# yc015/fully-automated-multi-heartbeat-echocardiography-video-segmentation-and-motion-tracking

Measured on AMD Instinct MI355X. Metric: 32f×112×112 clips/sec at 1/2/4/8 MI355X; Dice Δ vs CPU ref, higher is better.
Workload: dtype fp32

## Files before the change

### fully-automated-multi-heartbeat-echocardiography-video-segmentation-and-motion-tracking_amd/_lib.py

```python
import ctypes
import os

from .build import LIB_PATH

c_int, c_int64, c_void_p, c_char_p = ctypes.c_int, ctypes.c_int64, ctypes.c_void_p, ctypes.c_char_p
_P = c_void_p

SIGNATURES = {
    "clasfv_last_error": (c_char_p, []),
    "clasfv_version": (c_int, []),
    "clasfv_source_hash": (c_char_p, []),
    "clasfv_create": (c_int, [c_int, ctypes.POINTER(c_void_p)]),
    "clasfv_destroy": (c_int, [_P]),
    "clasfv_param_count": (c_int, [_P]),
    "clasfv_param_info": (c_int, [_P, c_int, ctypes.POINTER(c_char_p), ctypes.POINTER(c_int), ctypes.POINTER(c_int64)]),
    "clasfv_load_param": (c_int, [_P, c_char_p, _P, c_int64]),
    "clasfv_finalize": (c_int, [_P]),
    "clasfv_forward": (c_int, [_P, _P, c_int, c_int, c_int, c_int, _P, _P, _P]),
    "clasfv_workspace_bytes": (c_int64, [_P]),
    "clasfv_set_compute_dtype": (c_int, [_P, c_int]),
    "clasfv_get_compute_dtype": (c_int, [_P]),
    "clasfv_set_kernel_variants": (c_int, [_P, c_int]),
    "clasfv_get_kernel_variants": (c_int, [_P]),
    "clasfv_set_kernel_timing": (c_int, [_P, c_int]),
    "clasfv_kernel_timing": (c_int, [_P, c_int, ctypes.POINTER(c_char_p), ctypes.POINTER(c_int),
                                     ctypes.POINTER(ctypes.c_double), ctypes.POINTER(ctypes.c_double),
                                     ctypes.POINTER(ctypes.c_double)]),
    "clasfv_set_launch_log": (c_int, [_P, c_int]),
    "clasfv_launch_log": (c_int, [_P, c_int, ctypes.POINTER(c_char_p), ctypes.POINTER(c_int64), ctypes.POINTER(c_int),
                                  ctypes.POINTER(c_int)]),
    "clasfv_fill_workspace": (c_int, [_P, c_int, _P]),
    "clasfv_conv_count": (c_int, [_P]),
    "clasfv_conv_info": (c_int, [_P, c_int, ctypes.POINTER(c_char_p), ctypes.POINTER(c_char_p), ctypes.POINTER(c_int),
                                 ctypes.POINTER(c_int), ctypes.POINTER(c_int), ctypes.POINTER(c_int),
                                 ctypes.POINTER(c_int), ctypes.POINTER(c_int), ctypes.POINTER(c_int)]),
    "clasfv_run_conv": (c_int, [_P, c_int, _P, c_int, c_int, c_int, c_int, _P, _P, c_int, c_int, c_int, _P, _P, c_int64,
                                ctypes.POINTER(c_char_p), _P]),
    "clasfv_run_decoder": (c_int, [_P, _P, _P, _P, _P, c_int, c_int, c_int, c_int, _P, _P, _P]),
    "clasfv_build_clips": (c_int, [_P, c_int, c_int, c_int, _P, c_int, c_int, _P, _P]),
    "clasfv_pass_labels": (c_int, [_P, c_int, _P, c_int, c_int, c_int, c_int, c_int, _P, _P]),
    "clasfv_pass_labels_margin": (c_int, [_P, c_int, _P, c_int, c_int, c_int, c_int, c_int, _P, _P]),
    "clasfv_logit_margin": (c_int, [_P, c_int, c_int, c_int, _P, _P]),
    "clasfv_fuse_votes": (c_int, [_P, c_int, c_int, c_int, c_int, c_int, c_int, _P, _P]),
    "clasfv_warp": (c_int, [_P, c_int, c_int, c_int, c_int, _P, c_int64, c_int64, _P, _P]),
    "clasfv_zeroone_workspace_bytes": (c_int64, []),
    "clasfv_zeroone_normalize": (c_int, [_P, c_int64, _P, _P]),
# ... 71 lines not shown
```

### fully-automated-multi-heartbeat-echocardiography-video-segmentation-and-motion-tracking_amd/csrc/common.h

```cpp
#pragma once
#include <hip/hip_runtime.h>
#include <stdint.h>

#include "clasfv.h"

typedef float f32x4 __attribute__((ext_vector_type(4)));
typedef float f32x2 __attribute__((ext_vector_type(2)));

__device__ inline float relu1(float x) { return __int_as_float(max(__float_as_int(x), 0)); }

__device__ inline f32x4 psub4(f32x4 a, f32x4 b) {
  const f32x2 alo = {a[0], a[1]}, ahi = {a[2], a[3]}, blo = {b[0], b[1]}, bhi = {b[2], b[3]};
  f32x2 lo, hi;
  asm("v_pk_add_f32 %0, %1, %2 neg_lo:[0,1] neg_hi:[0,1]" : "=v"(lo) : "v"(alo), "v"(blo));
  asm("v_pk_add_f32 %0, %1, %2 neg_lo:[0,1] neg_hi:[0,1]" : "=v"(hi) : "v"(ahi), "v"(bhi));
  return f32x4{lo[0], lo[1], hi[0], hi[1]};
}


struct FastDiv {
  unsigned m;
  int l;
};
inline FastDiv fast_div(unsigned d) {
// ... 25 lines not shown
  } while (0)
#define CLASFV_LAUNCH(kernel, grid, ...) CLASFV_LAUNCH_P(1, kernel, grid, __VA_ARGS__)

struct ConvParams {
  const void* x;
  const void* w;
  const float* bias;
  const void* res;
  void* y;
  int N, Ti, Hi, Wi, Cin;
  int To, Ho, Wo, Cout;
  int KT, KH, KW, st, sh, sw, pt, ph, pw;
  int K, Kp, M, relu;
  const void* zero;
  const void* x2;
  int Cin2;
  int stem;
  int in_bf16, out_bf16;
  int x_c8, y_c8;
  int vflags, patch_nt;
  float* part;
  int n_split;
};

struct DecTap {
  const float* p;
  int T, H, W;
  float st, sh, sw;
};

struct DecParams {
  DecTap tap[4];
  const float* b1;
  const float* w2;
  const void* w2x3;
  const float* b2;
  const float* wh;
  const float* bh;
  float* seg;
  float* mot;
  int N, T, H, W;
  int bf16;
  int x3;
  void* idx;
};
inline size_t decoder_index_bytes(int T, int H, int W) { return (size_t)4 * (T + H + W) * 16; }
// ... 53 lines not shown
```

### fully-automated-multi-heartbeat-echocardiography-video-segmentation-and-motion-tracking_amd/csrc/engine.hip

```cpp
#include <cxxabi.h>
#include <math.h>
#include <stdio.h>
#include <stdlib.h>
#include <string.h>

#include <string>
#include <unordered_map>
#include <vector>

#include "clasfv.h"
#include "common.h"
#include "plumbing.h"
#include "track.h"

namespace {

thread_local std::string g_err;

int fail(int code, const std::string& msg) {
  g_err = msg;
  return code;
}

#define HIP_TRY(expr)                                                                        \
// ... 136 lines not shown
  c.cout_p = c.role == PROJ ? c.cout : pad_channels(c.cout, bf16);
  c.K = c.kt * c.kh * c.kw * c.cin_p + c.cin2;
  c.Kp = round_up(c.K, c.in_bf16 ? 32 : 16);
  c.cout_alloc = c.cout_p;
}

Conv make_conv(Role role, const std::string& w, const std::string& bn, int cin, int cout, int kt, int kh, int kw,
               int st, int sh, int sw, int pt, int ph, int pw) {
  Conv c;
  c.role = role;
  c.w = w;
  c.bn = bn;
  c.cin = cin;
  c.cout = cout;
  c.kt = kt, c.kh = kh, c.kw = kw, c.st = st, c.sh = sh, c.sw = sw, c.pt = pt, c.ph = ph, c.pw = pw;
  layout_conv(c, false);
  return c;
}

int midplanes(int i, int o) { return (i * o * 27) / (i * 9 + 3 * o); }

struct Tuning {
  int vflags = 0, conv_nt = 0, patch_nt = 0;
};

}

struct clasfv_engine {
  int device = 0;
  std::vector<Param> params;
  std::unordered_map<std::string, int> index;
  std::vector<Conv> convs;
  Conv proj[5];
  float *b1 = nullptr, *w2 = nullptr, *b2 = nullptr, *wh = nullptr, *bh = nullptr;
  void* w2x3 = nullptr;
  bool ready = false;
  int dtype = CLASFV_DTYPE_FP32;
  Tuning tune;
  float* zero = nullptr;
  struct Ctx {
    hipStream_t stream = nullptr;
    char* arena = nullptr;
    size_t arena_bytes = 0;
    hipStream_t side = nullptr;
    hipEvent_t ev_fork = nullptr, ev_join = nullptr;
    uint64_t last_use = 0;
// ... 456 lines not shown

bool c8_pair(const Conv& a, const Conv& b, const Shape5& in, const Tuning& tu) {
  if (tu.vflags & CLASFV_VARIANT_NO_C8) return false;
  Shape5 mid, out;
  ConvParams pa = conv_params(a, in, mid);
  ConvParams pb = conv_params(b, mid, out);
  pa.vflags = pb.vflags = tu.vflags;
  return kKernels[pick_kernel(a, pa)].writes_c8 && !a.out_bf16 && kKernels[pick_kernel(b, pb)].reads_c8 &&
         winot_c8_ok(pb);
}

void split_k(ConvParams& p, int S, void* scratch, size_t scratch_bytes) {
  if (S > 1 && scratch && (size_t)S * p.M * p.Cout * sizeof(float) <= scratch_bytes) {
    p.part = reinterpret_cast<float*>(scratch);
    p.n_split = S;
  }
}

int run_conv(const Conv& c, const void* x, const Shape5& in, void* y, Shape5& out, const void* res, bool relu,
             hipStream_t s, const void* zero_block, const void* x2, const KernelInfo** kernel, const Tuning& tu,
             int x_c8 = 0, int y_c8 = 0, void* scratch = nullptr, size_t scratch_bytes = 0) {
  if (in.c != c.cin_p) return fail(CLASFV_EINVAL, "internal: channel mismatch");
  ConvParams p = conv_params(c, in, out);
  p.vflags = tu.vflags;
  p.patch_nt = tu.patch_nt;
  p.x = x;
  p.res = res;
  p.y = y;
  p.relu = relu ? 1 : 0;
  p.zero = zero_block;
  p.x2 = x2;
  p.x_c8 = x_c8;
  p.y_c8 = y_c8;
  const KernelInfo& k = kKernels[pick_kernel(c, p)];
  *kernel = &k;
  if ((y_c8 && !k.writes_c8) || (x_c8 && !k.reads_c8))
    return fail(CLASFV_EINVAL, "internal: 8-channel-blocked layout on an unsupported kernel");
  p.w = c.*k.image;
  switch (k.id) {
    case K_WINO4R: HIP_TRY(launch_wino4r(p, s)); break;
    case K_WINO4W: HIP_TRY(launch_wino4w(p, s)); break;
    case K_WINO4: HIP_TRY(launch_wino4(p, s)); break;
    case K_WINO_Q: HIP_TRY(launch_winoq(p, s)); break;
    case K_WINO: HIP_TRY(launch_wino(p, s)); break;
    case K_STEM_BF16: HIP_TRY(launch_stem_bf16(p, s)); break;
    case K_STEM_X3: HIP_TRY(launch_stem_x3(p, s)); break;
    case K_WINOT:
// ... 202 lines not shown
    h->log.push_back({it->second.c_str(), r.e[i].grid, r.e[i].passes, conv});
  }
}

}

extern "C" {

const char* clasfv_last_error(void) { return g_err.c_str(); }
int clasfv_version(void) { return CLASFV_ABI_VERSION; }
#ifndef CLASFV_SOURCE_HASH
#define CLASFV_SOURCE_HASH "unhashed"
#endif
const char* clasfv_source_hash(void) { return "clasfv-source-hash:" CLASFV_SOURCE_HASH; }

int clasfv_create(int device, clasfv_t* out) {
  if (!out) return fail(CLASFV_EINVAL, "null out");
  int n = 0;
  HIP_TRY(hipGetDeviceCount(&n));
  if (device < 0 || device >= n) return fail(CLASFV_EINVAL, "bad device index");
  auto* e = new clasfv_engine();
  e->device = device;
  e->tune.vflags = env_variants();
  e->tune.conv_nt = env_int("CLASFV_CONV_NT");
  e->tune.patch_nt = env_int("CLASFV_PATCH_NT");
  build_plan(e);
  *out = e;
  return CLASFV_OK;
}

int clasfv_destroy(clasfv_t h) {
  if (!h) return CLASFV_OK;
  DeviceGuard guard(h->device);
  for (auto& c : h->convs) free_conv_images(c);
  for (auto& c : h->proj) free_conv_images(c);
  for (auto* c : h->ctxs) {
    if (c->side) (void)hipStreamDestroy(c->side);
    if (c->ev_fork) (void)hipEventDestroy(c->ev_fork);
    if (c->ev_join) (void)hipEventDestroy(c->ev_join);
    (void)hipFree(c->arena);
    delete c;
  }
  (void)hipFree(h->b1);
  (void)hipFree(h->w2);
  (void)hipFree(h->w2x3);
  (void)hipFree(h->b2);
// ... 67 lines not shown
}

int clasfv_set_compute_dtype(clasfv_t h, int dtype) {
  if (!h) return fail(CLASFV_EINVAL, "null handle");
  if (dtype != CLASFV_DTYPE_FP32 && dtype != CLASFV_DTYPE_BF16) return fail(CLASFV_EINVAL, "unknown dtype");
  if (dtype != h->dtype) {
    h->dtype = dtype;
    h->ready = false;
  }
  return CLASFV_OK;
}

int clasfv_get_compute_dtype(clasfv_t h) { return h ? h->dtype : CLASFV_EINVAL; }

int clasfv_set_kernel_variants(clasfv_t h, int flags) {
  if (!h) return fail(CLASFV_EINVAL, "null handle");
  if (flags & ~kVariantMask) return fail(CLASFV_EINVAL, "unknown kernel-variant bit");
  if ((flags ^ h->tune.vflags) & CLASFV_VARIANT_NO_WINOGRAD) h->ready = false;
  h->tune.vflags = flags;
  return CLASFV_OK;
}

int clasfv_get_kernel_variants(clasfv_t h) { return h ? h->tune.vflags : CLASFV_EINVAL; }

int clasfv_forward(clasfv_t h, const float* x, int N, int T, int H, int W, float* seg, float* mot, void* stream) {
  if (!h) return fail(CLASFV_EINVAL, "null handle");
  if (!h->ready) return fail(CLASFV_ENOTREADY, "clasfv_finalize has not been called");
  if (!x || !seg || !mot) return fail(CLASFV_EINVAL, "null tensor");
  if (N < 1) return fail(CLASFV_EINVAL, "N must be >= 1");
  if (T < 8 || H < 16 || W < 16 || T % 8 || H % 16 || W % 16)
    return fail(CLASFV_EBADSHAPE, "shape must satisfy T % 8 == 0, H % 16 == 0, W % 16 == 0 (got T=" +
                                      std::to_string(T) + " H=" + std::to_string(H) + " W=" + std::to_string(W) + ")");
  hipStream_t s = (hipStream_t)stream;
  DEVICE_GUARD(h->device);
  Layout L;
  make_layout(N, T, H, W, L);
  clasfv_engine::Ctx* cx = nullptr;
  if (int rc_ = acquire_ctx(h, s, L.total, &cx)) return rc_;
  char* const arena = cx->arena;
  auto buf = [&](int b) { return reinterpret_cast<void*>(arena + L.off[b]); };
  int last_ev = h->ktime ? tick(h, s) : -1;
  auto timed = [&](const char* name, double gflop, double xgflop) {
    if (last_ev < 0) return;
    const int e = tick(h, s);
    if (e >= 0) h->recs.push_back({name, gflop, xgflop, last_ev, e});
    last_ev = e;
// ... 381 lines not shown
```

### fully-automated-multi-heartbeat-echocardiography-video-segmentation-and-motion-tracking_amd/csrc/winograd4w.hip

```cpp
#include <cstdio>
#include <cstdlib>
#include <type_traits>

#include "wino4_common.h"

namespace {

template <int NTN>
struct W4W {
  static constexpr int NV = 18 * NTN;
  static constexpr int UQ = NTN == 9 ? 14 : 9;
  static constexpr int NU = (NV + 4 * UQ - 1) / (4 * UQ) * UQ;
};

constexpr int W4W_ZT = 20;
constexpr int W4W_ZP = 16 * W4W_ZT + 4;
constexpr int W4W_ZBUF = 42 * W4W_ZP;

constexpr int W4W_NTA = 7;
__device__ inline void mfma_v(f32x4& c, float a, float b) {
  asm volatile("s_nop 1\n\tv_mfma_f32_16x16x4_f32 %0, %1, %2, %0" : "+v"(c) : "v"(a), "v"(b));
}
__device__ inline void w4w_drain() { asm volatile("s_nop 7\n\ts_nop 4" ::: "memory"); }

// ... 300 lines not shown
    }
  }
#ifdef CLASFV_KNOCKOUTS
  if constexpr ((KO & 512) != 0) {
    __builtin_amdgcn_s_waitcnt(0);
    __syncthreads();
    st_[3] = __builtin_amdgcn_s_memrealtime();
    if (tid == 0 && blockIdx.x < W4W_NSTAMP) {
      unsigned long long* o = g_w4w_stamps[blockIdx.x];
      o[0] = st_[0], o[1] = st_[1], o[2] = st_[2], o[3] = st_[3];
      o[8] = __builtin_amdgcn_s_getreg((4 << 0) | (0 << 6) | (31 << 11));
      o[9] = __builtin_amdgcn_s_getreg((20 << 0) | (0 << 6) | (31 << 11));
    }
  }
#endif
}

constexpr int W4R_WAVES = 12;
constexpr int W4R_THREADS = 64 * W4R_WAVES;
constexpr int W4R_DPW = 7;
constexpr int W4R_NR = 2;
constexpr int W4R_NZ = 3;
constexpr int W4R_LDS = W4R_NZ * W4W_ZBUF * 4;
constexpr int W4R_MAX_LNI = (W4R_LDS - 1024) / (W4R_NR * 1024);
static_assert(W4R_MAX_LNI <= W4R_WAVES * W4R_DPW && W4R_LDS <= 160 * 1024, "ring and planes fit LDS");

template <int NTN>
struct W4R {
  static constexpr int NV = 6 * NTN;
  static constexpr int UQ = NTN == 9 ? 7 : NTN == 5 ? 8 : 9;
  static constexpr int NU = (NV + 4 * UQ - 1) / (4 * UQ) * UQ;
};

template <int RH, int R>
__device__ inline f32x2 bt_row(const f32x2 (&e)[5]) {
  if constexpr (RH == 0) {
    if constexpr (R == 0) {
      return e[0] * 4.f - e[2] * 5.f + e[4];
    } else if constexpr (R == 1) {
      const f32x2 s = e[1] + e[2], u = e[3] + e[4];
      return u - s * 4.f;
    } else {
      const f32x2 d = e[1] - e[2], w = e[4] - e[3];
      return w + d * 4.f;
    }
  } else {
    if constexpr (R == 2) {
      return e[0] * 4.f - e[2] * 5.f + e[4];
    } else {
      const f32x2 x = e[3] - e[1], y = e[2] - e[0];
      if constexpr (R == 0)
        return x + y * 2.f;
      else
        return x - y * 2.f;
    }
  }
}

template <int NTN, bool C8, int KO = 0, bool RELU = true, int CPB = 1, bool NTS = false>
__global__ __launch_bounds__(W4R_THREADS) __attribute__((amdgpu_waves_per_eu(3, 3))) void conv_wino4r(ConvParams p,
                                                                                                       W4Geo g) {
  using WR = W4R<NTN>;
  constexpr int UQ = WR::UQ, NU = WR::NU, NV = WR::NV;
  __shared__ __align__(16) char smem[W4R_LDS];
  const int STAGE = g.LNI * 1024;
  char* sink = smem + W4R_NR * STAGE;

#ifdef CLASFV_KNOCKOUTS
  unsigned long long st_[4] = {0, 0, 0, 0};
  if constexpr ((KO & 512) != 0) st_[0] = __builtin_amdgcn_s_memrealtime();
#endif
  if (g.stagger > 0 && blockIdx.x < 256) {
    const int sg = (blockIdx.x >> 3) % g.stagger_groups;
    if (sg) {
      const unsigned long long t0 = __builtin_amdgcn_s_memrealtime(), dt = (unsigned long long)sg * g.stagger;
      while (__builtin_amdgcn_s_memrealtime() - t0 < dt) __builtin_amdgcn_s_sleep(8);
    }
  }
  const __amdgpu_buffer_rsrc_t xr = __builtin_amdgcn_make_buffer_rsrc(
      const_cast<void*>(p.x), (short)0, (int)((size_t)p.N * p.Ti * p.Hi * p.Wi * p.Cin * 4), 0x00020000);
  const int tid = threadIdx.x, lane = tid & 63;
  const int wid = __builtin_amdgcn_readfirstlane(tid >> 6);
  const int blk = xcd_swizzle4(blockIdx.x, gridDim.x);
  const int grp = fdiv(blk, g.fd_cob), cob = blk - grp * g.n_cob;
  const int rg = fdiv(grp, g.fd_gpr), gx = grp - rg * g.gpr;
  const int R0 = rg * g.TR, tx0 = gx * g.TC;
  const int H = p.Ho, W = p.Wo, C = p.Cin;
  const int nchunk = C >> 3;
  const int NT = g.TR * g.TC;
  const int wq = wid / 3, r = wid - 3 * wq, rh = wq >> 1, ch = wq & 1;

  unsigned d_off[W4R_DPW];
// ... 90 lines not shown
  };

  const __amdgpu_buffer_rsrc_t ur = __builtin_amdgcn_make_buffer_rsrc(
      const_cast<float*>(reinterpret_cast<const float*>(p.w) + ((size_t)cob * nchunk * W4R_WAVES + wid) * (NU * 256)),
      (short)0, nchunk * W4R_WAVES * NU * 256 * 4, 0x00020000);
  auto load_u = [&](int k, int gi) __attribute__((always_inline)) {
    return __builtin_bit_cast(f32x4, __builtin_amdgcn_raw_buffer_load_b128(
                                         ur, lane * 16, ((k < nchunk ? k : 0) * (W4R_WAVES * NU * 256) + gi * 256) * 4, 0));
  };

  f32x4 acc[NTN][3];
#pragma unroll
  for (int nt = 0; nt < NTN; ++nt)
#pragma unroll
    for (int jj = 0; jj < 3; ++jj) acc[nt][jj] = f32x4{0.f, 0.f, 0.f, 0.f};
  f32x4 u[UQ];
  f32x2 a[3];

#pragma unroll
  for (int d = 0; d < W4R_NR; ++d) {
    issue_raw(d, d);
    __builtin_amdgcn_sched_barrier(0);
  }
#pragma unroll
  for (int gi = 0; gi < UQ; ++gi) u[gi] = load_u(0, gi);
  __builtin_amdgcn_sched_barrier(0);
  static_assert(W4R_DPW + UQ <= 63, "vmcnt field");
  __builtin_amdgcn_s_waitcnt(vm_wait(W4R_DPW + UQ));
  __builtin_amdgcn_sched_barrier(0);
  if constexpr ((KO & 16) == 0) __builtin_amdgcn_s_barrier();
  __builtin_amdgcn_sched_barrier(0);
#ifdef CLASFV_KNOCKOUTS
  if constexpr ((KO & 512) != 0) st_[1] = __builtin_amdgcn_s_memrealtime();
#endif

  int k = 0;
#pragma unroll 1
  do {
    const int kc = k & 3, S = k >> 2, buf = S & 1;
    if (kc == 0 && k > 0) {
      __builtin_amdgcn_s_waitcnt(vm_wait(UQ));
      __builtin_amdgcn_sched_barrier(0);
      if constexpr ((KO & 16) == 0) __builtin_amdgcn_s_barrier();
      __builtin_amdgcn_sched_barrier(0);
      if constexpr ((KO & 8) == 0) {
        if (32 * (S + 1) < C) issue_raw(S + 1, buf ^ 1);
      }
    }
    __builtin_amdgcn_sched_barrier(0);
    transform(buf, kc, a);
    __builtin_amdgcn_sched_barrier(0);
#pragma unroll
    for (int gi = 0; gi < NU; ++gi) {
#pragma unroll
      for (int c = 0; c < 4; ++c) {
        const int m = 4 * gi + c;
        if (m < NV) {
// ... 115 lines not shown
#pragma unroll
  for (int rd = 0; rd < NRND; ++rd) {
    __builtin_amdgcn_sched_barrier(0);
    __syncthreads();
    const int nt_u = W4R_NZ * rd + ug;
    const bool live = ulive && nt_u < NTN;
    f32x4 P[6];
    if (live) read_unit(ug, P);
    if (rd + 1 < NRND) {
      __syncthreads();
#pragma unroll
      for (int b = 0; b < W4R_NZ; ++b)
        if (W4R_NZ * (rd + 1) + b < NTN) write_planes(W4R_NZ * (rd + 1) + b, b);
    }
    if (live) store_unit(nt_u, biasv[rd], P);
  }
#ifdef CLASFV_KNOCKOUTS
  if constexpr ((KO & 512) != 0) {
    __builtin_amdgcn_s_waitcnt(0);
    __syncthreads();
    st_[3] = __builtin_amdgcn_s_memrealtime();
    if (tid == 0 && blockIdx.x < W4W_NSTAMP) {
      unsigned long long* o = g_w4w_stamps[blockIdx.x];
      o[0] = st_[0], o[1] = st_[1], o[2] = st_[2], o[3] = st_[3];
      o[8] = __builtin_amdgcn_s_getreg((4 << 0) | (0 << 6) | (31 << 11));
      o[9] = __builtin_amdgcn_s_getreg((20 << 0) | (0 << 6) | (31 << 11));
    }
  }
#endif
}

template <int NTN, int KO = 0, int CPB = 1>
hipError_t launch_w4r(const ConvParams& p, const W4Geo& g, int n_blocks, hipStream_t s) {
  const dim3 grid(n_blocks), block(W4R_THREADS);
  if (!(p.vflags & CLASFV_VARIANT_W4R_CACHED_STORES)) {
    if (p.y_c8 && p.relu) {
      CLASFV_LAUNCH((conv_wino4r<NTN, true, KO, true, CPB, true>), grid, block, 0, s, p, g);
      return hipGetLastError();
    }
    if (p.relu) {
      CLASFV_LAUNCH((conv_wino4r<NTN, false, KO, true, CPB, true>), grid, block, 0, s, p, g);
      return hipGetLastError();
    }
  }
  if (p.y_c8 && p.relu)
    CLASFV_LAUNCH((conv_wino4r<NTN, true, KO, true, CPB>), grid, block, 0, s, p, g);
  else if (p.relu)
    CLASFV_LAUNCH((conv_wino4r<NTN, false, KO, true, CPB>), grid, block, 0, s, p, g);
  else if (p.y_c8)
    CLASFV_LAUNCH((conv_wino4r<NTN, true, KO, false, CPB>), grid, block, 0, s, p, g);
  else
    CLASFV_LAUNCH((conv_wino4r<NTN, false, KO, false, CPB>), grid, block, 0, s, p, g);
  return hipGetLastError();
}

constexpr int W4W_FILL = 1;

int wino4w_ntn(int cout) {
  if (cout % 16) return 0;
  for (int n : {9, 6})
    if ((cout / 16) % n == 0) return n;
  return 0;
}

template <int NTN, int DPW, int KO = 0>
hipError_t launch_w4w(const ConvParams& p, const W4Geo& g, int n_blocks, hipStream_t s) {
  const dim3 grid(n_blocks), block(W4_THREADS);
  if (p.y_c8 && p.relu)
    CLASFV_LAUNCH((conv_wino4w<NTN, true, DPW, KO, true>), grid, block, 0, s, p, g);
  else if (p.relu)
    CLASFV_LAUNCH((conv_wino4w<NTN, false, DPW, KO, true>), grid, block, 0, s, p, g);
  else if (p.y_c8)
    CLASFV_LAUNCH((conv_wino4w<NTN, true, DPW, KO, false>), grid, block, 0, s, p, g);
  else
    CLASFV_LAUNCH((conv_wino4w<NTN, false, DPW, KO, false>), grid, block, 0, s, p, g);
// ... 73 lines not shown
    }
}

int wino4r_ntn(int cout) {
  if (cout % 16) return 0;
  for (int n : {9, 6})
    if ((cout / 16) % n == 0) return n;
  return 0;
}

static int w4r_nu(int ntn) { return ntn == 9 ? W4R<9>::NU : ntn == 6 ? W4R<6>::NU : W4R<5>::NU; }

bool wino4r_supported(const ConvParams& p) {
  W4Geo g;
  int nb;
  const int ntn = wino4r_ntn(p.Cout);
  return ntn && !p.in_bf16 && !p.out_bf16 && !p.stem && !p.x2 && !p.res && p.KT == 1 && p.KH == 3 && p.KW == 3 &&
         p.sh == 1 && p.sw == 1 && p.st == 1 && p.ph == 1 && p.pw == 1 && p.pt == 0 && p.Ho == p.Hi &&
         p.Wo == p.Wi && p.To == p.Ti &&
         (size_t)p.N * p.To * p.Ho * p.Wo * (p.Cin > p.Cout ? p.Cin : p.Cout) < ((size_t)1 << 31) &&
         wino4_geometry(p, &g, &nb, 16 * ntn, W4W_FILL) && g.LNI <= W4R_MAX_LNI;
}

static void w4r_stagger(const ConvParams& p, int ntn, int n_blocks, W4Geo* g) {
  if (n_blocks < 16 * 256) return;
  g->stagger_groups = 8;
  g->stagger = (1370 + 264 * (p.Cin / 8) * ntn / 9) / 8;
}

hipError_t launch_wino4r(const ConvParams& p, hipStream_t s) {
  if (!wino4r_supported(p)) return hipErrorInvalidValue;
  W4Geo g;
  int nb;
  const int ntn = wino4r_ntn(p.Cout);
  wino4_geometry(p, &g, &nb, 16 * ntn, W4W_FILL);
  w4r_stagger(p, ntn, nb, &g);
  return ntn == 9 ? launch_w4r<9>(p, g, nb, s) : launch_w4r<6>(p, g, nb, s);
}

double wino4r_exec_gflop(const ConvParams& p) {
  W4Geo g;
  int nb;
  const int ntn = wino4r_ntn(p.Cout);
  return ntn && wino4_geometry(p, &g, &nb, 16 * ntn, W4W_FILL) ? 2.0 * nb * 16.0 * 36.0 * p.Cin * 16.0 * ntn * 1e-9 : 0.0;
}

size_t wino4r_weight_floats(int cin_p, int cout_p) {
  const int ntn = wino4r_ntn(cout_p);
  if (!ntn) return 0;
  return (size_t)(cout_p / (16 * ntn)) * (cin_p / 8) * W4R_WAVES * w4r_nu(ntn) * 256;
}

void wino4r_transform_weights(const double* w, int cout, int cin, int cout_p, int cin_p, float* U) {
  static const double G[6][3] = {{1.0 / 4, 0, 0},
                                 {-1.0 / 6, -1.0 / 6, -1.0 / 6},
                                 {-1.0 / 6, 1.0 / 6, -1.0 / 6},
                                 {1.0 / 24, 1.0 / 12, 1.0 / 6},
                                 {1.0 / 24, -1.0 / 12, 1.0 / 6},
                                 {0, 0, 1}};
// ... 28 lines not shown
  if (!wino4w_supported(p) || wino4w_ntn(p.Cout) != 9) return hipErrorInvalidValue;
  W4Geo g;
  int nb;
  wino4_geometry(p, &g, &nb, 144, (ko & 1024) ? 0 : (ko & 2048) ? 1 : W4W_FILL);
  ko &= ~3072;
  switch (ko) {
    case 1: return launch_w4w_dpw<9, 1>(p, g, nb, s);
    case 2: return launch_w4w_dpw<9, 2>(p, g, nb, s);
    case 4: return launch_w4w_dpw<9, 4>(p, g, nb, s);
    case 8: return launch_w4w_dpw<9, 8>(p, g, nb, s);
    case 15: return launch_w4w_dpw<9, 15>(p, g, nb, s);
    case 128: return launch_w4w_dpw<9, 128>(p, g, nb, s);
    case 256: return launch_w4w_dpw<9, 256>(p, g, nb, s);
    case 512: return launch_w4w_dpw<9, 512>(p, g, nb, s);
    default: return launch_w4w_dpw<9>(p, g, nb, s);
  }
}
hipError_t launch_wino4r_ko(const ConvParams& p, hipStream_t s, int ko) {
  if (!wino4w_supported(p) || wino4w_ntn(p.Cout) != 9) return hipErrorInvalidValue;
  W4Geo g;
  int nb;
  wino4_geometry(p, &g, &nb, 144, W4W_FILL);
  if (const char* e = getenv("CB_W4R_STAGGER")) sscanf(e, "%d,%d", &g.stagger, &g.stagger_groups);
  switch (ko) {
    case 1: return launch_w4r<9, 1>(p, g, nb, s);
    case 2: return launch_w4r<9, 2>(p, g, nb, s);
    case 8: return launch_w4r<9, 8>(p, g, nb, s);
    case 16: return launch_w4r<9, 16>(p, g, nb, s);
    case 31: return launch_w4r<9, 31>(p, g, nb, s);
    case 4: return launch_w4r<9, 4>(p, g, nb, s);
    case 128: return launch_w4r<9, 128>(p, g, nb, s);
    case 512: return launch_w4r<9, 512>(p, g, nb, s);
    case 32: return launch_w4r<9, 0, 2>(p, g, nb, s);
    case 96: return launch_w4r<9, 0, 3>(p, g, nb, s);
    case 160: return launch_w4r<9, 0, 0>(p, g, nb, s);
    case 2048: return launch_w4r<9, 2048>(p, g, nb, s);
    default: return launch_w4r<9>(p, g, nb, s);
  }
}
void wino4r_from_wino4w(const float* Uw, int cin_p, int cout_p, float* Ur) {
  const int ntn = wino4w_ntn(cout_p);
  const int nuw = ntn == 9 ? W4W<9>::NU : W4W<6>::NU, nur = ntn == 9 ? W4R<9>::NU : W4R<6>::NU;
  const int nch = cin_p / 8, ncob = cout_p / (16 * ntn);
  for (size_t i = 0; i < wino4r_weight_floats(cin_p, cout_p); ++i) Ur[i] = 0.f;
  for (int cob = 0; cob < ncob; ++cob)
    for (int ck = 0; ck < nch; ++ck)
// ... 13 lines not shown
```

### fully-automated-multi-heartbeat-echocardiography-video-segmentation-and-motion-tracking_amd/model.py

```python
import ctypes
import warnings
from collections import OrderedDict

import numpy as np
import torch
from torch import nn

from . import _lib
from .arch import strip_module_prefix
from .weights import DEFAULT_SEED, recipe_state_dict


class Engine:

    def __init__(self, device=None, dtype="fp32"):
        if not torch.cuda.is_available():
            raise RuntimeError("CLAS-FV engine requires a HIP (ROCm) GPU; none is visible")
        self.lib = _lib.load()
        self.device = torch.device("cuda", torch.cuda.current_device() if device is None else
                                   torch.device(device).index or 0)
        h = ctypes.c_void_p()
        _lib.check(self.lib.clasfv_create(self.device.index, ctypes.byref(h)), "clasfv_create")
        self.h = h
        self.set_dtype(dtype)

    def set_dtype(self, dtype):
        if dtype not in _lib.DTYPES:
            raise ValueError(f"dtype must be one of {sorted(_lib.DTYPES)}")
        _lib.check(self.lib.clasfv_set_compute_dtype(self.h, _lib.DTYPES[dtype]), "clasfv_set_compute_dtype")
        self.dtype = "bf16" if _lib.DTYPES[dtype] == 1 else "fp32"

    def set_variants(self, *names):
        flags = 0
        for n in names:
            if n not in _lib.VARIANTS:
                raise ValueError(f"unknown kernel variant {n!r}: {sorted(_lib.VARIANTS)}")
            flags |= _lib.VARIANTS[n]
        old = self.lib.clasfv_get_kernel_variants(self.h)
        _lib.check(self.lib.clasfv_set_kernel_variants(self.h, flags), "clasfv_set_kernel_variants")
        return tuple(n for n, b in _lib.VARIANTS.items() if old & b)

    def __del__(self):
        try:
            if getattr(self, "h", None):
                self.lib.clasfv_destroy(self.h)
                self.h = None
        except Exception:
            pass

    def param_table(self):
        out = []
        name = ctypes.c_char_p()
        nd = ctypes.c_int()
        dims = (ctypes.c_int64 * 5)()
        for i in range(self.lib.clasfv_param_count(self.h)):
            _lib.check(self.lib.clasfv_param_info(self.h, i, ctypes.byref(name), ctypes.byref(nd), dims), "param_info")
            out.append((name.value.decode(), tuple(int(dims[d]) for d in range(nd.value))))
        return out

    def load(self, state):
        for k, v in state.items():
            a = np.ascontiguousarray(np.asarray(v.detach().cpu() if torch.is_tensor(v) else v), dtype=np.float32)
            _lib.check(self.lib.clasfv_load_param(self.h, k.encode(), a.ctypes.data_as(ctypes.c_void_p), a.size),
# ... 147 lines not shown
```

### include/clasfv.h

```cpp
#ifndef CLASFV_H
#define CLASFV_H

#include <stdint.h>

#ifdef __cplusplus
extern "C" {
#endif

enum {
  CLASFV_OK = 0,
  CLASFV_EINVAL = -1,
  CLASFV_EBADSHAPE = -2,
  CLASFV_ENOTREADY = -3,
  CLASFV_EHIP = -4,
  CLASFV_ENOMEM = -5
};

#define CLASFV_ABI_VERSION 3

enum { CLASFV_FUSE_MAJORITY = 0, CLASFV_FUSE_SIMPLE = 1, CLASFV_FUSE_STAPLE = 2, CLASFV_FUSE_ITKVOTING = 3 };
#define CLASFV_FUSE_FORCE_GENERIC 0x100
enum { CLASFV_DTYPE_FP32 = 0, CLASFV_DTYPE_BF16 = 1 };

enum {
// ... 21 lines not shown
  CLASFV_VARIANT_NO_TWALK = 67108864
};

typedef struct clasfv_engine* clasfv_t;

const char* clasfv_last_error(void);
int clasfv_version(void);
const char* clasfv_source_hash(void);

int clasfv_create(int device, clasfv_t* out);
int clasfv_destroy(clasfv_t h);
int clasfv_param_count(clasfv_t h);
int clasfv_param_info(clasfv_t h, int i, const char** name, int* ndim, int64_t dims[5]);
int clasfv_load_param(clasfv_t h, const char* name, const float* host_data, int64_t numel);
int clasfv_finalize(clasfv_t h);
int clasfv_forward(clasfv_t h, const float* x_dev, int N, int T, int H, int W, float* seg_dev,
                   float* motion_dev, void* stream);
int64_t clasfv_workspace_bytes(clasfv_t h);
int clasfv_set_compute_dtype(clasfv_t h, int dtype);
int clasfv_get_compute_dtype(clasfv_t h);
int clasfv_set_kernel_variants(clasfv_t h, int flags);
int clasfv_get_kernel_variants(clasfv_t h);

int clasfv_set_kernel_timing(clasfv_t h, int enable);
int clasfv_kernel_timing(clasfv_t h, int cap, const char** names, int* launches, double* ms,
                         double* gflop, double* xgflop);

int clasfv_set_launch_log(clasfv_t h, int enable);
int clasfv_launch_log(clasfv_t h, int cap, const char** labels, int64_t* grids, int* passes, int* convs);
int clasfv_fill_workspace(clasfv_t h, int byte, void* stream);

int clasfv_conv_count(clasfv_t h);
int clasfv_conv_info(clasfv_t h, int i, const char** prefix, const char** bn_prefix, int* tap, int channels[5],
                     int kernel[3], int stride[3], int padding[3], int* in_dtype, int* out_dtype);
int clasfv_run_conv(clasfv_t h, int i, const void* x_dev, int N, int T, int H, int W, const void* x2_dev,
                    const void* res_dev, int relu, int x_c8, int y_c8, void* y_dev, void* scratch_dev,
                    int64_t scratch_bytes, const char** kernel_name, void* stream);
int clasfv_run_decoder(clasfv_t h, const float* p01_dev, const float* p2_dev, const float* p3_dev,
                       const float* p4_dev, int N, int T, int H, int W, float* seg_dev, float* motion_dev,
                       void* stream);

int clasfv_build_clips(const float* video_dev, int T, int H, int W, const int32_t* table_dev, int n,
                       int interpolate, float* clips_dev, void* stream);
int clasfv_pass_labels(const float* logits_dev, int K, const int32_t* pass_clip0, int T, int step, int H,
                       int W, int interpolate, uint8_t* labels_dev, void* stream);
int clasfv_pass_labels_margin(const float* margin_dev, int K, const int32_t* pass_clip0, int T, int step,
// ... 32 lines not shown
```

Measured before the change: 1467.

## Add three-pass Winograd F(4,3) wino4r path for Cin=64, 144-output-channel convs

For convolutions with Cin=64 and NTN=9, the wino4r kernel now keeps the transformed input chunks (xc) in registers. It then computes the 144 output channels in three passes of 48, each with its own accumulators, overlapping each pass's epilogue (LDS plane writes, output transform, stores) with the next pass's MFMAs. The goal is to cut accumulator register pressure and hide epilogue latency behind matrix work, and stagger is disabled for this path. It is on by default and can be turned off with an env var or API call. It adds complex scheduling and extra barriers, and it reissues weight loads for each pass.

```diff
diff --git a/fully-automated-multi-heartbeat-echocardiography-video-segmentation-and-motion-tracking_amd/_lib.py b/fully-automated-multi-heartbeat-echocardiography-video-segmentation-and-motion-tracking_amd/_lib.py
--- a/fully-automated-multi-heartbeat-echocardiography-video-segmentation-and-motion-tracking_amd/_lib.py
+++ b/fully-automated-multi-heartbeat-echocardiography-video-segmentation-and-motion-tracking_amd/_lib.py
@@ -22,6 +22,7 @@
     "clasfv_get_compute_dtype": (c_int, [_P]),
     "clasfv_set_kernel_variants": (c_int, [_P, c_int]),
     "clasfv_get_kernel_variants": (c_int, [_P]),
+    "clasfv_set_w4r_one_pass": (c_int, [_P, c_int]),
     "clasfv_set_kernel_timing": (c_int, [_P, c_int]),
     "clasfv_kernel_timing": (c_int, [_P, c_int, ctypes.POINTER(c_char_p), ctypes.POINTER(c_int),
                                      ctypes.POINTER(ctypes.c_double), ctypes.POINTER(ctypes.c_double),
diff --git a/fully-automated-multi-heartbeat-echocardiography-video-segmentation-and-motion-tracking_amd/csrc/common.h b/fully-automated-multi-heartbeat-echocardiography-video-segmentation-and-motion-tracking_amd/csrc/common.h
--- a/fully-automated-multi-heartbeat-echocardiography-video-segmentation-and-motion-tracking_amd/csrc/common.h
+++ b/fully-automated-multi-heartbeat-echocardiography-video-segmentation-and-motion-tracking_amd/csrc/common.h
@@ -71,6 +71,8 @@
   float* part;
   int n_split;
 };
+
+constexpr int W4R_VFLAG_ONE_PASS = 1 << 30;
 
 struct DecTap {
   const float* p;
diff --git a/fully-automated-multi-heartbeat-echocardiography-video-segmentation-and-motion-tracking_amd/csrc/engine.hip b/fully-automated-multi-heartbeat-echocardiography-video-segmentation-and-motion-tracking_amd/csrc/engine.hip
--- a/fully-automated-multi-heartbeat-echocardiography-video-segmentation-and-motion-tracking_amd/csrc/engine.hip
+++ b/fully-automated-multi-heartbeat-echocardiography-video-segmentation-and-motion-tracking_amd/csrc/engine.hip
@@ -182,6 +182,7 @@
 
 struct Tuning {
   int vflags = 0, conv_nt = 0, patch_nt = 0;
+  int w4r_one_pass = 0;
 };
 
 }
@@ -684,7 +685,7 @@
              int x_c8 = 0, int y_c8 = 0, void* scratch = nullptr, size_t scratch_bytes = 0) {
   if (in.c != c.cin_p) return fail(CLASFV_EINVAL, "internal: channel mismatch");
   ConvParams p = conv_params(c, in, out);
-  p.vflags = tu.vflags;
+  p.vflags = tu.vflags | (tu.w4r_one_pass ? W4R_VFLAG_ONE_PASS : 0);
   p.patch_nt = tu.patch_nt;
   p.x = x;
   p.res = res;
@@ -933,6 +934,7 @@
   auto* e = new clasfv_engine();
   e->device = device;
   e->tune.vflags = env_variants();
+  e->tune.w4r_one_pass = getenv("CLASFV_W4R_ONE_PASS") ? 1 : 0;
   e->tune.conv_nt = env_int("CLASFV_CONV_NT");
   e->tune.patch_nt = env_int("CLASFV_PATCH_NT");
   build_plan(e);
@@ -1046,6 +1048,13 @@
 }
 
 int clasfv_get_kernel_variants(clasfv_t h) { return h ? h->tune.vflags : CLASFV_EINVAL; }
+
+int clasfv_set_w4r_one_pass(clasfv_t h, int enable) {
+  if (!h) return fail(CLASFV_EINVAL, "null handle");
+  const int old = h->tune.w4r_one_pass;
+  h->tune.w4r_one_pass = enable ? 1 : 0;
+  return old;
+}
 
 int clasfv_forward(clasfv_t h, const float* x, int N, int T, int H, int W, float* seg, float* mot, void* stream) {
   if (!h) return fail(CLASFV_EINVAL, "null handle");
diff --git a/fully-automated-multi-heartbeat-echocardiography-video-segmentation-and-motion-tracking_amd/csrc/winograd4w.hip b/fully-automated-multi-heartbeat-echocardiography-video-segmentation-and-motion-tracking_amd/csrc/winograd4w.hip
--- a/fully-automated-multi-heartbeat-echocardiography-video-segmentation-and-motion-tracking_amd/csrc/winograd4w.hip
+++ b/fully-automated-multi-heartbeat-echocardiography-video-segmentation-and-motion-tracking_amd/csrc/winograd4w.hip
@@ -346,6 +346,8 @@
 constexpr int W4R_NR = 2;
 constexpr int W4R_NZ = 3;
 constexpr int W4R_LDS = W4R_NZ * W4W_ZBUF * 4;
+constexpr int W4R_PASSES_CPB = 0;
+constexpr int W4R_PG = 5;
 constexpr int W4R_MAX_LNI = (W4R_LDS - 1024) / (W4R_NR * 1024);
 static_assert(W4R_MAX_LNI <= W4R_WAVES * W4R_DPW && W4R_LDS <= 160 * 1024, "ring and planes fit LDS");
 
@@ -381,17 +383,17 @@
   }
 }
 
-template <int NTN, bool C8, int KO = 0, bool RELU = true, int CPB = 1, bool NTS = false>
+template <int NTN, bool C8, int KO = 0, bool RELU = true, int CPB = 1, bool NTS = false, bool PASSES = false>
 __global__ __launch_bounds__(W4R_THREADS) __attribute__((amdgpu_waves_per_eu(3, 3))) void conv_wino4r(ConvParams p,
                                                                                                        W4Geo g) {
   using WR = W4R<NTN>;
-  constexpr int UQ = WR::UQ, NU = WR::NU, NV = WR::NV;
+  constexpr int UQ = PASSES ? W4R_PG : WR::UQ, NU = WR::NU, NV = WR::NV;
   __shared__ __align__(16) char smem[W4R_LDS];
   const int STAGE = g.LNI * 1024;
   char* sink = smem + W4R_NR * STAGE;
 
 #ifdef CLASFV_KNOCKOUTS
-  unsigned long long st_[4] = {0, 0, 0, 0};
+  unsigned long long st_[6] = {0, 0, 0, 0, 0, 0};
   if constexpr ((KO & 512) != 0) st_[0] = __builtin_amdgcn_s_memrealtime();
 #endif
   if (g.stagger > 0 && blockIdx.x < 256) {
@@ -528,8 +530,16 @@
     issue_raw(d, d);
     __builtin_amdgcn_sched_barrier(0);
   }
-#pragma unroll
-  for (int gi = 0; gi < UQ; ++gi) u[gi] = load_u(0, gi);
+  f32x4 uq[4];
+  f32x2 uh;
+  if constexpr (PASSES) {
+#pragma unroll
+    for (int gi = 0; gi < 4; ++gi) uq[gi] = load_u(0, gi);
+    uh = __builtin_bit_cast(f32x2, __builtin_amdgcn_raw_buffer_load_b64(ur, lane * 16, 4 * 256 * 4, 0));
+  } else {
+#pragma unroll
+    for (int gi = 0; gi < UQ; ++gi) u[gi] = load_u(0, gi);
+  }
   __builtin_amdgcn_sched_barrier(0);
   static_assert(W4R_DPW + UQ <= 63, "vmcnt field");
   __builtin_amdgcn_s_waitcnt(vm_wait(W4R_DPW + UQ));
@@ -539,6 +549,260 @@
 #ifdef CLASFV_KNOCKOUTS
   if constexpr ((KO & 512) != 0) st_[1] = __builtin_amdgcn_s_memrealtime();
 #endif
+
+  if constexpr (PASSES) {
+    static_assert(NTN == 9 && W4R_NZ == 3 && UQ == W4R_PG, "three passes of one epilogue round each");
+    constexpr int NCH = 8;
+    constexpr int CB = 1, CS = 2;
+    constexpr int LGKM0 = 0xC07F;
+    using I1 = std::integral_constant<int, 1>;
+    using I2 = std::integral_constant<int, 2>;
+    const int slot = wid >> 2;
+    float* Z0 = reinterpret_cast<float*>(smem);
+    const int q = lane >> 4, l16 = lane & 15;
+    const size_t plane = (size_t)p.N * p.To * H * W * 8;
+    float* yout = reinterpret_cast<float*>(p.y);
+    const int ug = tid >> 8, ut = tid & 255;
+    const int ub = ut & 3, ucq = (ut >> 2) & 3, utile = ut >> 4;
+    const int useg = fdiv(utile, g.fd_tc), utc = utile - useg * g.TC;
+    const int uR = R0 + useg, uf = fdiv(uR, g.fd_th), uty = uR - uf * g.TH;
+    const int uxx = 4 * (tx0 + utc) + ub;
+    const bool ulive = utile < NT && uxx < W;
+    const int eb = ub == 3 ? 1 : ub;
+    const int CO = p.Cout;
+    const int zrow = 3 * rh + r;
+    auto write_planes = [&](const f32x4 (&m)[3], int buf) __attribute__((always_inline)) {
+      float* Z = Z0 + buf * W4W_ZBUF;
+      const f32x4 m0 = m[0], m1 = m[1], m2 = m[2];
+      if (ch == 0) {
+        f32x4* zp = reinterpret_cast<f32x4*>(Z + (zrow * 3) * W4W_ZP + l16 * W4W_ZT + 4 * q);
+        zp[0] = m0 + m1 + m2;
+        zp[W4W_ZP / 4] = psub4(m1, m2);
+        zp[2 * W4W_ZP / 4] = m1 + m2;
+      } else {
+        f32x4* zp = reinterpret_cast<f32x4*>(Z + (18 + zrow * 4) * W4W_ZP + l16 * W4W_ZT + 4 * q);
+        const f32x4 sm = m0 + m1, df = psub4(m0, m1);
+        zp[0] = sm;
+        zp[W4W_ZP / 4] = 2.f * df;
+        zp[2 * W4W_ZP / 4] = 4.f * sm;
+        zp[3 * W4W_ZP / 4] = 8.f * df + m2;
+      }
+    };
+    auto read_unit = [&](int buf, f32x4 (&P)[6]) __attribute__((always_inline)) {
+      const float* Z = Z0 + buf * W4W_ZBUF;
+#pragma unroll
+      for (int i = 0; i < 6; ++i)
+        P[i] = *reinterpret_cast<const f32x4*>(Z + (i * 3 + eb) * W4W_ZP + utile * W4W_ZT + 4 * ucq) +
+               *reinterpret_cast<const f32x4*>(Z + (18 + i * 4 + ub) * W4W_ZP + utile * W4W_ZT + 4 * ucq);
+    };
+    const int co0 = cob * NTN * 16 + 4 * ucq;
+    const size_t upix = (size_t)(uf * H + 4 * uty) * W + uxx;
+    float* const y0 = yout + (C8 ? (size_t)(co0 >> 3) * plane + upix * 8 + (co0 & 7) : upix * CO + co0);
+    const size_t row_step = C8 ? (size_t)W * 8 : (size_t)W * CO;
+    const size_t nt_step = C8 ? 2 * plane : 16;
+    const __amdgpu_buffer_rsrc_t br = __builtin_amdgcn_make_buffer_rsrc(const_cast<float*>(p.bias), (short)0,
+                                                                        p.bias ? p.Cout * 4 : 0, 0x00020000);
+    auto load_bias = [&](int rd) __attribute__((always_inline)) {
+      return __builtin_bit_cast(f32x4, __builtin_amdgcn_raw_buffer_load_b128(br, (co0 + (W4R_NZ * rd + ug) * 16) * 4, 0, 0));
+    };
+    auto store_unit = [&](int nt, const f32x4& bias, const f32x4 (&P)[6]) __attribute__((always_inline)) {
+      const f32x4 s12 = P[1] + P[2], d12 = psub4(P[1], P[2]), s34 = P[3] + P[4], d34 = psub4(P[3], P[4]);
+      f32x4 y[4];
+      y[0] = P[0] + s12 + s34;
+      y[1] = d12 + 2.f * d34;
+      y[2] = s12 + 4.f * s34;
+      y[3] = d12 + 8.f * d34 + P[5];
+#pragma unroll
+      for (int aa = 0; aa < 4; ++aa) {
+        if (4 * uty + aa >= H) break;
+        f32x4 o = y[aa] + bias;
+        if constexpr (RELU) {
+#pragma unroll
+          for (int c = 0; c < 4; ++c) o[c] = relu1(o[c]);
+        }
+        float* dst = y0 + aa * row_step + nt * nt_step;
+        if constexpr ((KO & 128) != 0) {
+          if (o[0] == 1234.5f) *reinterpret_cast<f32x4*>(dst) = o;
+        } else if constexpr (NTS || (KO & 2048) != 0) {
+          __builtin_nontemporal_store(o, reinterpret_cast<f32x4*>(dst));
+        } else {
+          *reinterpret_cast<f32x4*>(dst) = o;
+        }
+      }
+    };
+    auto wg_barrier = [&]() __attribute__((always_inline)) {
+      __builtin_amdgcn_sched_barrier(0);
+      __builtin_amdgcn_s_waitcnt(LGKM0);
+      __builtin_amdgcn_s_barrier();
+      __builtin_amdgcn_sched_barrier(0);
+    };
+
+    auto load_q = [&](int k, int gi) __attribute__((always_inline)) { return load_u(k, gi); };
+    auto load_h = [&](int k, int gi, int half) __attribute__((always_inline)) {
+      return __builtin_bit_cast(f32x2, __builtin_amdgcn_raw_buffer_load_b64(
+                                           ur, lane * 16, (k * (W4R_WAVES * NU * 256) + gi * 256) * 4 + half * 8, 0));
+    };
+    auto u_val = [&](int ps, int ml) __attribute__((always_inline)) {
+      if (ps == 1) return ml < 2 ? uh[ml] : uq[(ml - 2) >> 2][(ml - 2) & 3];
+      return ml < 16 ? uq[ml >> 2][ml & 3] : uh[ml - 16];
+    };
+    f32x4 acc3[3][3];
+    f32x2 xc[NCH][3];
+#pragma unroll
+    for (int nt = 0; nt < 3; ++nt)
+#pragma unroll
+      for (int jj = 0; jj < 3; ++jj) acc3[nt][jj] = f32x4{0.f, 0.f, 0.f, 0.f};
+    float kosum = 0.f;
+    (void)kosum;
+
+    auto mfma0 = [&](const f32x2 (&ac)[3], int kn, int gb, bool last) __attribute__((always_inline)) {
+#pragma unroll
+      for (int ml = 0; ml < 18; ++ml) {
+        const int jj = ml % 3, ks = (ml / 3) % 2, nt = ml / 6;
+        acc3[nt][jj] = __builtin_amdgcn_mfma_f32_16x16x4f32(u_val(0, ml), ks ? ac[jj].y : ac[jj].x, acc3[nt][jj], 0, 0, 0);
+        if constexpr ((KO & 2) == 0) {
+          if (ml % 4 == 3) uq[ml / 4] = load_q(kn, gb + ml / 4);
+          if (ml == 17) uh = load_h(kn, 4, last ? 1 : 0);
+        }
+      }
+    };
+    int k = 0;
+#pragma unroll 1
+    do {
+      if (k == 4) {
+        __builtin_amdgcn_s_waitcnt(vm_wait(UQ));
+        __builtin_amdgcn_sched_barrier(0);
+        if constexpr ((KO & 16) == 0) __builtin_amdgcn_s_barrier();
+        __builtin_amdgcn_sched_barrier(0);
+      }
+      __builtin_amdgcn_sched_barrier(0);
+      transform(k >> 2, k & 3, a);
+      __builtin_amdgcn_sched_barrier(0);
+      const bool last = k + 1 == NCH;
+      mfma0(a, last ? 0 : k + 1, last ? 5 : 0, last);
+#pragma unroll
+      for (int gi = 0; gi < W4R_PG; ++gi) {
+        if (gi < 4)
+          __builtin_amdgcn_sched_group_barrier(0x008, 4, 0);
+        else
+          __builtin_amdgcn_sched_group_barrier(0x008, 2, 0);
+        if constexpr ((KO & 2) == 0) __builtin_amdgcn_sched_group_barrier(0x020, 1, 0);
+      }
+      __builtin_amdgcn_sched_barrier(0);
+#pragma unroll
+      for (int kk = 0; kk < NCH; ++kk)
+        if (k == kk) {
+#pragma unroll
+          for (int jj = 0; jj < 3; ++jj) xc[kk][jj] = a[jj];
+          asm volatile("" : "+v"(xc[kk][0]), "+v"(xc[kk][1]), "+v"(xc[kk][2]));
+        }
+    } while (++k < NCH);
+    wg_barrier();
+#ifdef CLASFV_KNOCKOUTS
+    if constexpr ((KO & 512) != 0) st_[4] = __builtin_amdgcn_s_memrealtime();
+#endif
+
+    f32x4 biasv;
+    auto pass = [&](auto ps_c) __attribute__((always_inline)) {
+      constexpr int PS = decltype(ps_c)::value, QB = PS == 1 ? 5 : 9, HG = PS == 1 ? 4 : 13, HH = PS == 1 ? 1 : 0;
+      if constexpr ((KO & 4) == 0) {
+        biasv = load_bias(PS - 1);
+#pragma unroll
+        for (int b = 0; b < 3; ++b) write_planes(acc3[b], b);
+      } else {
+#pragma unroll
+        for (int nt = 0; nt < 3; ++nt)
+#pragma unroll
+          for (int jj = 0; jj < 3; ++jj) kosum += acc3[nt][jj][0] + acc3[nt][jj][3];
+      }
+#pragma unroll
+      for (int nt = 0; nt < 3; ++nt)
+#pragma unroll
+        for (int jj = 0; jj < 3; ++jj) acc3[nt][jj] = f32x4{0.f, 0.f, 0.f, 0.f};
+#pragma unroll
+      for (int kk = 0; kk < NCH; ++kk) {
+        __builtin_amdgcn_sched_barrier(0);
+        if constexpr ((KO & 4) == 0) {
+          if (kk == CB) wg_barrier();
+#pragma unroll
+          for (int sl = 0; sl < 3; ++sl)
+            if (kk == CS + sl) {
+              if (slot == sl && ulive) {
+                f32x4 P[6];
+                read_unit(ug, P);
+                store_unit(W4R_NZ * (PS - 1) + ug, biasv, P);
+              }
+              __builtin_amdgcn_sched_barrier(0);
+            }
+        }
+        if constexpr ((KO & 4) == 0 && PS == 2)
+          if (kk == NCH - 1) biasv = load_bias(2);
+        const bool reload = (KO & 2) == 0 && (kk + 1 < NCH || PS == 1);
+        const int kn = kk + 1 < NCH ? kk + 1 : 0, qb = kk + 1 < NCH ? QB : 9, hg = kk + 1 < NCH ? HG : 13;
+        const int hh = kk + 1 < NCH ? HH : 0;
+#pragma unroll
+        for (int ml = 0; ml < 18; ++ml) {
+          const int jj = ml % 3, ks = (ml / 3) % 2, nt = ml / 6;
+          acc3[nt][jj] =
+              __builtin_amdgcn_mfma_f32_16x16x4f32(u_val(PS, ml), ks ? xc[kk][jj].y : xc[kk][jj].x, acc3[nt][jj], 0, 0, 0);
+          if (reload) {
+            if (PS == 1) {
+              if (ml == 1) uh = load_h(kn, hg, hh);
+              if (ml >= 2 && (ml - 2) % 4 == 3) uq[(ml - 2) / 4] = load_q(kn, qb + (ml - 2) / 4);
+            } else {
+              if (ml % 4 == 3) uq[ml / 4] = load_q(kn, qb + ml / 4);
+              if (ml == 17) uh = load_h(kn, hg, hh);
+            }
+          }
+        }
+#pragma unroll
+        for (int gi = 0; gi < W4R_PG; ++gi) {
+          if (PS == 1 ? gi == 0 : gi == 4)
+            __builtin_amdgcn_sched_group_barrier(0x008, 2, 0);
+          else
+            __builtin_amdgcn_sched_group_barrier(0x008, 4, 0);
+          if (reload) __builtin_amdgcn_sched_group_barrier(0x020, 1, 0);
+        }
+      }
+      if constexpr ((KO & 4) == 0) wg_barrier();
+#ifdef CLASFV_KNOCKOUTS
+      if constexpr ((KO & 512) != 0) st_[PS == 1 ? 5 : 2] = __builtin_amdgcn_s_memrealtime();
+#endif
+    };
+    pass(I1{});
+    pass(I2{});
+
+    if constexpr ((KO & 4) != 0) {
+#pragma unroll
+      for (int nt = 0; nt < 3; ++nt)
+#pragma unroll
+        for (int jj = 0; jj < 3; ++jj) kosum += acc3[nt][jj][0] + acc3[nt][jj][3];
+      if (kosum == 1234.5f) reinterpret_cast<float*>(p.y)[tid] = kosum;
+    } else {
+#pragma unroll
+      for (int b = 0; b < 3; ++b) write_planes(acc3[b], b);
+      wg_barrier();
+      if (ulive) {
+        f32x4 P[6];
+        read_unit(ug, P);
+        store_unit(W4R_NZ * 2 + ug, biasv, P);
+      }
+    }
+#ifdef CLASFV_KNOCKOUTS
+    if constexpr ((KO & 512) != 0) {
+      __builtin_amdgcn_s_waitcnt(0);
+      __syncthreads();
+      st_[3] = __builtin_amdgcn_s_memrealtime();
+      if (tid == 0 && blockIdx.x < W4W_NSTAMP) {
+        unsigned long long* o = g_w4w_stamps[blockIdx.x];
+        o[0] = st_[0], o[1] = st_[1], o[2] = st_[2], o[3] = st_[3], o[4] = st_[4], o[5] = st_[5];
+        o[8] = __builtin_amdgcn_s_getreg((4 << 0) | (0 << 6) | (31 << 11));
+        o[9] = __builtin_amdgcn_s_getreg((20 << 0) | (0 << 6) | (31 << 11));
+      }
+    }
+#endif
+    return;
+  }
 
   int k = 0;
 #pragma unroll 1
@@ -700,7 +964,7 @@
     st_[3] = __builtin_amdgcn_s_memrealtime();
     if (tid == 0 && blockIdx.x < W4W_NSTAMP) {
       unsigned long long* o = g_w4w_stamps[blockIdx.x];
-      o[0] = st_[0], o[1] = st_[1], o[2] = st_[2], o[3] = st_[3];
+      o[0] = st_[0], o[1] = st_[1], o[2] = st_[2], o[3] = st_[3], o[4] = st_[4], o[5] = st_[5];
       o[8] = __builtin_amdgcn_s_getreg((4 << 0) | (0 << 6) | (31 << 11));
       o[9] = __builtin_amdgcn_s_getreg((20 << 0) | (0 << 6) | (31 << 11));
     }
@@ -708,27 +972,27 @@
 #endif
 }
 
-template <int NTN, int KO = 0, int CPB = 1>
+template <int NTN, int KO = 0, int CPB = 1, bool PASSES = false>
 hipError_t launch_w4r(const ConvParams& p, const W4Geo& g, int n_blocks, hipStream_t s) {
   const dim3 grid(n_blocks), block(W4R_THREADS);
   if (!(p.vflags & CLASFV_VARIANT_W4R_CACHED_STORES)) {
     if (p.y_c8 && p.relu) {
-      CLASFV_LAUNCH((conv_wino4r<NTN, true, KO, true, CPB, true>), grid, block, 0, s, p, g);
+      CLASFV_LAUNCH((conv_wino4r<NTN, true, KO, true, CPB, true, PASSES>), grid, block, 0, s, p, g);
       return hipGetLastError();
     }
     if (p.relu) {
-      CLASFV_LAUNCH((conv_wino4r<NTN, false, KO, true, CPB, true>), grid, block, 0, s, p, g);
+      CLASFV_LAUNCH((conv_wino4r<NTN, false, KO, true, CPB, true, PASSES>), grid, block, 0, s, p, g);
       return hipGetLastError();
     }
   }
   if (p.y_c8 && p.relu)
-    CLASFV_LAUNCH((conv_wino4r<NTN, true, KO, true, CPB>), grid, block, 0, s, p, g);
+    CLASFV_LAUNCH((conv_wino4r<NTN, true, KO, true, CPB, false, PASSES>), grid, block, 0, s, p, g);
   else if (p.relu)
-    CLASFV_LAUNCH((conv_wino4r<NTN, false, KO, true, CPB>), grid, block, 0, s, p, g);
+    CLASFV_LAUNCH((conv_wino4r<NTN, false, KO, true, CPB, false, PASSES>), grid, block, 0, s, p, g);
   else if (p.y_c8)
-    CLASFV_LAUNCH((conv_wino4r<NTN, true, KO, false, CPB>), grid, block, 0, s, p, g);
+    CLASFV_LAUNCH((conv_wino4r<NTN, true, KO, false, CPB, false, PASSES>), grid, block, 0, s, p, g);
   else
-    CLASFV_LAUNCH((conv_wino4r<NTN, false, KO, false, CPB>), grid, block, 0, s, p, g);
+    CLASFV_LAUNCH((conv_wino4r<NTN, false, KO, false, CPB, false, PASSES>), grid, block, 0, s, p, g);
   return hipGetLastError();
 }
 
@@ -848,10 +1112,15 @@
          wino4_geometry(p, &g, &nb, 16 * ntn, W4W_FILL) && g.LNI <= W4R_MAX_LNI;
 }
 
-static void w4r_stagger(const ConvParams& p, int ntn, int n_blocks, W4Geo* g) {
+static void w4r_stagger(const ConvParams& p, int ntn, int n_blocks, bool passes, W4Geo* g) {
   if (n_blocks < 16 * 256) return;
+  if (passes) return;
   g->stagger_groups = 8;
   g->stagger = (1370 + 264 * (p.Cin / 8) * ntn / 9) / 8;
+}
+
+static bool w4r_passes(const ConvParams& p, int ntn) {
+  return ntn == 9 && p.Cin == 64 && !(p.vflags & W4R_VFLAG_ONE_PASS);
 }
 
 hipError_t launch_wino4r(const ConvParams& p, hipStream_t s) {
@@ -860,7 +1129,9 @@
   int nb;
   const int ntn = wino4r_ntn(p.Cout);
   wino4_geometry(p, &g, &nb, 16 * ntn, W4W_FILL);
-  w4r_stagger(p, ntn, nb, &g);
+  const bool passes = w4r_passes(p, ntn);
+  w4r_stagger(p, ntn, nb, passes, &g);
+  if (passes) return launch_w4r<9, 0, W4R_PASSES_CPB, true>(p, g, nb, s);
   return ntn == 9 ? launch_w4r<9>(p, g, nb, s) : launch_w4r<6>(p, g, nb, s);
 }
 
@@ -935,6 +1206,21 @@
   int nb;
   wino4_geometry(p, &g, &nb, 144, W4W_FILL);
   if (const char* e = getenv("CB_W4R_STAGGER")) sscanf(e, "%d,%d", &g.stagger, &g.stagger_groups);
+  if (w4r_passes(p, 9)) {
+    switch (ko) {
+      case 1: return launch_w4r<9, 1, W4R_PASSES_CPB, true>(p, g, nb, s);
+      case 4: return launch_w4r<9, 4, W4R_PASSES_CPB, true>(p, g, nb, s);
+      case 128: return launch_w4r<9, 128, W4R_PASSES_CPB, true>(p, g, nb, s);
+      case 512: return launch_w4r<9, 512, W4R_PASSES_CPB, true>(p, g, nb, s);
+      case 0: return launch_w4r<9, 0, W4R_PASSES_CPB, true>(p, g, nb, s);
+      case 224: return launch_w4r<9, 0, 1, true>(p, g, nb, s);
+      case 32: return launch_w4r<9, 0, 2, true>(p, g, nb, s);
+      case 96: return launch_w4r<9, 0, 3, true>(p, g, nb, s);
+      case 192: return launch_w4r<9, 0, 6, true>(p, g, nb, s);
+      case 160: return launch_w4r<9, 0, 0, true>(p, g, nb, s);
+      default: return hipErrorInvalidValue;
+    }
+  }
   switch (ko) {
     case 1: return launch_w4r<9, 1>(p, g, nb, s);
     case 2: return launch_w4r<9, 2>(p, g, nb, s);
diff --git a/fully-automated-multi-heartbeat-echocardiography-video-segmentation-and-motion-tracking_amd/model.py b/fully-automated-multi-heartbeat-echocardiography-video-segmentation-and-motion-tracking_amd/model.py
--- a/fully-automated-multi-heartbeat-echocardiography-video-segmentation-and-motion-tracking_amd/model.py
+++ b/fully-automated-multi-heartbeat-echocardiography-video-segmentation-and-motion-tracking_amd/model.py
@@ -39,6 +39,12 @@
         old = self.lib.clasfv_get_kernel_variants(self.h)
         _lib.check(self.lib.clasfv_set_kernel_variants(self.h, flags), "clasfv_set_kernel_variants")
         return tuple(n for n, b in _lib.VARIANTS.items() if old & b)
+
+    def set_w4r_one_pass(self, enable=True):
+        old = self.lib.clasfv_set_w4r_one_pass(self.h, 1 if enable else 0)
+        if old < 0:
+            _lib.check(old, "clasfv_set_w4r_one_pass")
+        return bool(old)
 
     def __del__(self):
         try:
diff --git a/include/clasfv.h b/include/clasfv.h
--- a/include/clasfv.h
+++ b/include/clasfv.h
@@ -67,6 +67,8 @@
 int clasfv_set_kernel_variants(clasfv_t h, int flags);
 int clasfv_get_kernel_variants(clasfv_t h);
 
+int clasfv_set_w4r_one_pass(clasfv_t h, int enable);
+
 int clasfv_set_kernel_timing(clasfv_t h, int enable);
 int clasfv_kernel_timing(clasfv_t h, int cap, const char** names, int* launches, double* ms,
                          double* gflop, double* xgflop);
```

Result: no change. 1474 (median of 2 runs) (+0.4%).
